# eboigne/PyTV-4D

Measured on AMD Instinct MI355X. Metric: chambolle_pock_iters_per_sec, higher is better.
Workload: dtype f32

## Files before the change

### pytv-4d_amd/csrc/tv_fused.h

```cpp
#pragma once
#include "tv_device.h"
#include "tv_stencil.h"

namespace tv {

using F4 = Vec<float, 4>;

#ifndef TV_FUSED_TR
#define TV_FUSED_TR 8
#endif
#ifndef TV_FUSED_NW
#define TV_FUSED_NW 8
#endif
#ifndef TV_ADMM_T_NT
#define TV_ADMM_T_NT 0
#endif
#ifndef TV_FUSED_PFQ_TWIN
#define TV_FUSED_PFQ_TWIN 1
#endif
#ifndef TV_FUSED_PFQ
#define TV_FUSED_PFQ 2
#endif
#ifndef TV_FUSED_PFX
#define TV_FUSED_PFX 1
// ... 644 lines not shown
    return vload_s<T, V>(p);
#else
    return vload<T, V>(p);
#endif
}
template <typename T, int V> __device__ __forceinline__ void FXST(T* p, const Vec<T, V>& a) {
#if TV_FIXUP_NT
    vstore_s<T, V>(p, a);
#else
    vstore<T, V>(p, a);
#endif
}
template <int S, bool XW, typename T = float, int ALG = ALG_CP>
__device__ __forceinline__ double fixup_site(const DG& g, const WT<T>& w, const FixupArgsT<T>& a, int zchunk, int zl, int t, int y,
                                             int col0) {
    constexpr int V = 16 / (int)sizeof(T);
    using VT = Vec<T, V>;
    constexpr bool UP = (S != DOWNWIND), DN = (S != UPWIND), CEN = (S == CENTRAL);
    if (!fused_needs_fixup<S, XW, V>(g, zl, y, col0, zchunk, t)) return 0.0;
    constexpr int CM = XW ? CPG<V>::BC - 1 : CPG<V>::WC - 1;
    const int c_ru = 0, c_cu = 1, c_rd = (S == HYBRID) ? 2 : 0, c_cd = (S == HYBRID) ? 3 : 1;
    const int c_zu = g.ch_z, c_zd = (S == HYBRID) ? g.ch_z + 1 : g.ch_z;
    const bool z_fwd = CEN && g.z_two;
    const long long inpl = (long long)t * g.s_t + (long long)y * g.rp + col0;
    const T* qb = a.q + (long long)zl * g.s_dz + inpl;
    const VT zero = vsplat<T, V>(T(0));
    VT m = zero;
    if (UP && (y & (CP_TR - 1)) == 0 && y >= (CEN ? 2 : 1)) m = m + FXLD<T, V>(qb + (long long)c_ru * g.s_z - g.rp);
    if (DN && (y & (CP_TR - 1)) == CP_TR - 1 && y <= g.ny - (CEN ? 3 : 2)) m = m - FXLD<T, V>(qb + (long long)c_rd * g.s_z + g.rp);
    if (UP && (col0 & CM) == 0 && col0 >= (CEN ? 2 : 1)) m.v[0] += qb[(long long)c_cu * g.s_z - 1];
    if (DN && (col0 & CM) == CM - (V - 1) && col0 + V <= g.nx - (CEN ? 2 : 1)) m.v[V - 1] -= qb[(long long)c_cd * g.s_z + V];
    if (g.za) {
        const int gz = g.z0 + zl;
        const int zs = (zl / zchunk) * zchunk;
        const int ze = (zs + zchunk < g.nz) ? zs + zchunk : g.nz;
        if (UP && zl == zs && gz >= ((CEN && !z_fwd) ? 2 : 1)) {
            const VT u = (zl >= 1) ? FXLD<T, V>(qb + (long long)c_zu * g.s_z - g.s_dz) : FXLD<T, V>(a.qp + inpl);
            m = m + w.wz * u;
        }
        if (DN && !z_fwd && zl == ze - 1 && gz <= g.nzg - (CEN ? 3 : 2)) {
            const VT d = (zl + 1 < g.nz) ? FXLD<T, V>(qb + (long long)c_zd * g.s_z + g.s_dz) : FXLD<T, V>(a.qn + inpl);
            m = m - w.wz * d;
        }
    }
    if (g.ta && g.m > CP_TWN) {
        const int c_tu = g.ch_t, c_td = (S == HYBRID) ? g.ch_t + 1 : g.ch_t;
        const int k = t % CP_TWN;
        VT mt = zero;
        if (UP && k == 0 && t >= 1) mt = mt + FXLD<T, V>(qb + (long long)c_tu * g.s_z - g.s_t) * vol_factor<T, V>(g, zl, t - 1, y, col0);
        if (DN && k == CP_TWN - 1 && t <= g.m - (CEN ? 3 : 2))
            mt = mt - FXLD<T, V>(qb + (long long)c_td * g.s_z + g.s_t) * vol_factor<T, V>(g, zl, t + 1, y, col0);
        m = m + (w.wt * mt) * mask_factor<T, V>(g, w.sf, y, col0);
    }
    const T s = (S == HYBRID) ? Consts<T>::inv_sqrt2() : (CEN ? T(0.5) : T(1));
    const long long off = (long long)zl * g.s_z + inpl;
    const VT xv = FXLD<T, V>(a.x_out + off);
    VT x0v = zero;
    if constexpr (ALG == ALG_CP) { if (a.x0 != nullptr) x0v = FXLD<T, V>(a.x0 + off); }
    VT xo;
    double acc = 0.0;
#pragma unroll
    for (int i = 0; i < V; ++i) {
        xo.v[i] = xv.v[i] - a.tau * (s * m.v[i]);
        const double e = (double)xo.v[i] - (double)x0v.v[i];
        acc += (ALG == ALG_CP ? 0.5 : 1.0) * e * e;
    }
    FXST<T, V>(a.x_out + off, xo);
    return acc;
}

template <int S> __device__ __forceinline__ bool is_fix_row(const DG& g, int y) {
    constexpr bool UP = (S != DOWNWIND), DN = (S != UPWIND);
    return (UP && (y & (CP_TR - 1)) == 0 && y >= 1) || (DN && (y & (CP_TR - 1)) == CP_TR - 1 && y <= g.ny - 2);
}
template <int S> __device__ __forceinline__ bool is_fix_plane(const DG& g, int zl, int zchunk) {
    constexpr bool UP = (S != DOWNWIND), DN = (S != UPWIND);
    if (!g.za) return false;
    const int gz = g.z0 + zl;
    const int zs = (zl / zchunk) * zchunk;
    const int ze = (zs + zchunk < g.nz) ? zs + zchunk : g.nz;
    return (UP && zl == zs && gz >= 1) || (DN && zl == ze - 1 && gz <= g.nzg - 2);
}

template <int S, int CLS, bool XW, typename T = float, int ALG = ALG_CP>
__global__ __launch_bounds__(256) void k_cp_fixup(DG g, WT<T> w, FixupArgsT<T> a, int zchunk, int zb, int zn, double* partials) {
    constexpr int V = 16 / (int)sizeof(T);
    __shared__ double sm[16];
    const int nxv = (g.nx + V - 1) / V;
    const int tiles_x = (nxv + 63) / 64;
    double acc = 0.0;
    if (CLS == 0) {
        const int bx = (int)blockIdx.x % tiles_x, grp = (int)blockIdx.x / tiles_x;
        const int ty = (int)threadIdx.y;
        int y;
        if (S == HYBRID || S == CENTRAL) y = grp * 2 * CP_TR + ((ty & 1) ? CP_TR - 1 : 0) + ((ty & 2) ? CP_TR : 0);
        else y = grp * 4 * CP_TR + CP_TR * ty + (S == DOWNWIND ? CP_TR - 1 : 0);
        const int col0 = (bx * 64 + (int)threadIdx.x) * V;
        if (col0 < g.nx && y < g.ny && is_fix_row<S>(g, y) && !is_seam_frame<S>(g, (int)blockIdx.y))
            acc = fixup_site<S, XW, T, ALG>(g, w, a, zchunk, zb + (int)blockIdx.z, (int)blockIdx.y, y, col0);
    } else if (CLS == 1) {
        const int k = (int)blockIdx.z, chunk = a.chunk0 + (k >> 1);
        const int zs = chunk * zchunk;
        const int ze = (zs + zchunk < g.nz) ? zs + zchunk : g.nz;
        const int zl = (k & 1) ? ze - 1 : zs;
        const bool dup = (k & 1) && (ze - 1 == zs);
        const int bx = (int)blockIdx.x % tiles_x, by = (int)blockIdx.x / tiles_x;
        const int y = by * 4 + (int)threadIdx.y;
        const int col0 = (bx * 64 + (int)threadIdx.x) * V;
        if (!dup && zs < g.nz && zl >= zb && zl < zb + zn && col0 < g.nx && y < g.ny && is_fix_plane<S>(g, zl, zchunk) &&
            !is_fix_row<S>(g, y) && !is_seam_frame<S>(g, (int)blockIdx.y))
            acc = fixup_site<S, XW, T, ALG>(g, w, a, zchunk, zl, (int)blockIdx.y, y, col0);
    } else if (CLS == 3) {
        const int wdw = (int)blockIdx.y >> 1, t = wdw * CP_TWN + (((int)blockIdx.y & 1) ? CP_TWN - 1 : 0);
        const int bx = (int)blockIdx.x % tiles_x, by = (int)blockIdx.x / tiles_x;
        const int y = by * 4 + (int)threadIdx.y;
        const int col0 = (bx * 64 + (int)threadIdx.x) * V;
        if (t < g.m && col0 < g.nx && y < g.ny && is_seam_frame<S>(g, t))
            acc = fixup_site<S, XW, T, ALG>(g, w, a, zchunk, zb + (int)blockIdx.z, t, y, col0);
    } else {
        constexpr int TW = XW ? CPG<V>::BC : CPG<V>::WC;
        const int ntile = (g.nx + TW - 1) / TW, ncand = 2 * ntile;
        const long long idx = (long long)blockIdx.x * 256 + (int)threadIdx.y * 64 + (int)threadIdx.x;
        const int zl = zb + (int)blockIdx.z;
        if (idx < (long long)g.ny * ncand && !is_fix_plane<S>(g, zl, zchunk) && !is_seam_frame<S>(g, (int)blockIdx.y)) {
            const int y = (int)(idx / ncand), cnd = (int)(idx % ncand);
            const int col0 = (cnd >> 1) * TW + ((cnd & 1) ? TW - V : 0);
            if (col0 < g.nx && !is_fix_row<S>(g, y)) acc = fixup_site<S, XW, T, ALG>(g, w, a, zchunk, zl, (int)blockIdx.y, y, col0);
        }
    }
    acc = block_sum(acc, sm);
    if (threadIdx.x == 0 && threadIdx.y == 0) partials[linear_block_id()] = acc;
}


template <int S, int M>
__global__ __launch_bounds__(256, 2) void k_subgrad_march(DG g, WT<float> w, const float* __restrict__ x, const float* __restrict__ xp,
                                                          const float* __restrict__ xn, const float* __restrict__ norms_ext,
                                                          float* __restrict__ G, int zchunk) {
    static_assert(S != CENTRAL, "radius-2 scheme");
    constexpr bool UP = (S == UPWIND || S == HYBRID), DN = (S == DOWNWIND || S == HYBRID);
    const FusedCoord c = fused_coord(g, zchunk, 0);
    const F4 zero = vsplat<float, 4>(0.f), one = vsplat<float, 4>(1.f);
    const F4 mf = g.ta ? mask_factor<float, 4>(g, w.sf, c.ok ? c.y : 0, c.ok ? c.col0 : 0) : one;
    __shared__ F4 lds_WC[M][256];
    __shared__ F4 lds_WP[M][256];
    const int tid = (int)threadIdx.y * 64 + (int)threadIdx.x;
    auto nplane = [&](int zl) -> const float* {
        const int gz = g.z0 + zl;
        return (gz >= 0 && gz < g.nzg) ? norms_ext + (long long)(zl + 1) * g.s_z : nullptr;
    };
    F4 XC[M], XP[M];
    {
        const float* pc = zplane<float>(g, x, xp, xn, 2, c.zs);
        const float* pp = g.za ? zplane<float>(g, x, xp, xn, 2, c.zs - 1) : nullptr;
        const float* qc = nplane(c.zs);
        const float* qp = g.za ? nplane(c.zs - 1) : nullptr;
#pragma unroll
        for (int t = 0; t < M; ++t) {
            const long long off = (long long)t * g.s_t + c.inpl;
            XC[t] = c.ok ? vload<float, 4>(pc + off) : zero;
            XP[t] = (c.ok && pp) ? vload<float, 4>(pp + off) : zero;
            lds_WC[t][tid] = c.ok ? vload<float, 4>(qc + off) : one;
            lds_WP[t][tid] = (c.ok && qp && UP) ? vload<float, 4>(qp + off) : one;
        }
    }
    auto neighbourhood = [&](XN<float, 4>& n, const F4& cv, const float* plane_c, long long off, const F4& nzv, const F4& pzv,
                             const F4& ntv, const F4& ptv, bool h_nz, bool h_pz, bool h_nt, bool h_pt) {
        n.c = cv;
        n.col0 = c.col0;
        const bool want_up = (c.row == 0) && c.ok && (c.y > 0);
        const bool want_dn = (c.row == 3) && c.ok && (c.y + 1 < g.ny);
        F4 halo = zero;
        if (want_up || want_dn) halo = vload<float, 4>(plane_c + off + (want_up ? -(long long)g.rp : (long long)g.rp));
        n.h_nr = c.ok && (c.y + 1 < g.ny);
        n.h_pr = c.ok && (c.y > 0);
        const F4 sdn = shfl_down16(cv), sup = shfl_up16(cv);
        n.nr = (c.row == 3) ? halo : sdn;
        n.pr = (c.row == 0) ? halo : sup;
        const bool le = (c.lx == 0) && c.ok && (c.col0 > 0), re = (c.lx == 15) && c.ok && (c.col0 + 4 < g.nx);
        float edge = 0.f;
        if (le || re) edge = le ? plane_c[off - 1] : plane_c[off + 4];
        const float shr = __shfl_down(cv.v[0], 1, 64), shl = __shfl_up(cv.v[3], 1, 64);
        n.nc = shift_left<float, 4>(cv, (c.lx == 15) ? edge : shr);
        n.pc = shift_right<float, 4>(cv, (c.lx == 0) ? edge : shl);
        n.nz = nzv; n.pz = pzv; n.nt = ntv; n.pt = ptv;
        n.h_nz = h_nz; n.h_pz = h_pz; n.h_nt = h_nt; n.h_pt = h_pt;
    };
    for (int z = c.zs; z < c.ze; ++z) {
        const int gz = g.z0 + z;
        const float* pc = zplane<float>(g, x, xp, xn, 2, z);
        const float* pn = zplane<float>(g, x, xp, xn, 2, z + 1);
        const float* qc = nplane(z);
        const float* qn = nplane(z + 1);
        const bool has_pz = g.za && (gz > 0), has_nz = g.za && (pn != nullptr);
        const bool more = (z + 1 < c.ze);
        F4 xcold = zero, wcold = one;
#pragma unroll
        for (int t = 0; t < M; ++t) {
            const long long off = (long long)t * g.s_t + c.inpl;
            const F4 XNv = (pn != nullptr && c.ok && (has_nz || more)) ? vload<float, 4>(pn + off) : zero;
            const F4 WNv = (qn != nullptr && c.ok && ((has_nz && DN) || more)) ? vload<float, 4>(qn + off) : one;
            const F4 wc = lds_WC[t][tid], wp = lds_WP[t][tid];
            const bool h_nt = g.ta && (t + 1 < M), h_pt = g.ta && (t > 0);
            XN<float, 4> xs, ns;
            neighbourhood(xs, XC[t], pc, off, XNv, XP[t], XC[(t + 1 < M) ? t + 1 : t], xcold, has_nz, has_pz, h_nt, h_pt);
            neighbourhood(ns, wc, qc, off, WNv, wp, lds_WC[(t + 1 < M) ? t + 1 : t][tid], wcold, has_nz, has_pz, h_nt, h_pt);
            if (c.ok) {
                const F4 r = subgrad_site<S, float, 4>(g, w, xs, ns, mf);
                vstore<float, 4>(G + (long long)z * g.s_z + off, r);
            }
            xcold = XC[t];
            wcold = wc;
            XP[t] = XC[t];
            XC[t] = XNv;
// ... 8 lines not shown
```

### pytv-4d_amd/csrc/tv_fused.hip

```cpp
#include "tv_fused_launch.h"

TV_FUSED_INSTANTIATE(float, ALG_CP)

static int fused_zchunk(const DG& d) {
    int zc = env_int("TV_ZCHUNK", 0);
    if (zc <= 0) {
        const long long nwin = (d.m > CP_TWN) ? (d.m + CP_TWN - 1) / CP_TWN : 1;
        const long long tiles = (long long)(((d.nx + d.vl - 1) / d.vl + CP_NW * CP_TL - 1) / (CP_NW * CP_TL)) * ((d.ny + CP_TR - 1) / CP_TR) * nwin;
        const long long want = (1024 + tiles - 1) / (tiles > 0 ? tiles : 1);
        zc = (int)(d.nz / (want > 0 ? want : 1));
        if (zc > 32) zc = 32;
        if (zc < 8) zc = 8;
        while (zc > 2 && tiles * ((d.nz + zc - 1) / zc) < 256) zc -= 2;
        if (d.nz < d.nzg) {
            const int q4 = (int)(d.nz / 4);
            if (zc > q4) zc = q4 < 4 ? 4 : q4;
        }
    }
    if (zc < 1) zc = 1;
    if (zc > d.nz) zc = (int)d.nz;
    return zc;
}

namespace tvm {
bool subgrad_pass2_ok(const tv_geom* g, const DG& d) { return g->scheme != TV_CENTRAL && d.m >= 1 && d.m <= 8; }
int subgrad_pass2(const tv_geom* g, const DG& d, const void* x, const void* xp, const void* xn, hipStream_t st,
                  const float* norms_ext, float* G) {
    const int zc = march_zchunk(d);
    const LC lc = march_cfg(d, zc);
    return dispatch_scheme_m(WindowedMs{}, g->scheme, d.m, kNoFusedSM, [&]<int S, int M>() -> int {
        if constexpr (S != CENTRAL && M >= 1) {
            hipLaunchKernelGGL((k_subgrad_march<S, M>), lc.grid, lc.block, 0, st, d, make_w<float>(g), (const float*)x,
                               (const float*)xp, (const float*)xn, norms_ext, G, zc);
            HIP_TRY(hipGetLastError());
            return 0;
        } else {
            return fail(TV_E_ARG, "central: radius-2 gather, not a marching kernel");
        }
    });
}
}

struct SweepPlan {
    LC lc;
    int zc, chunk0;
    bool xw, force_win;
};
static int sweep_plan(const tv_geom* g, const DG& d, const Partials& P, const void* x_in, const void* x_prev, const void* x_next,
                      int64_t chunk_begin, int64_t chunk_count, SweepPlan& sp, bool& empty) {
    sp.zc = fused_zchunk(d);
    const int zc = sp.zc;
    {
        const long long nch_all = (d.nz + zc - 1) / zc;
        const long long cb = (chunk_count < 0) ? 0 : chunk_begin, ce = (chunk_count < 0) ? nch_all : chunk_begin + chunk_count;
        const bool first = (cb == 0 && ce > 0), last = (ce == nch_all && ce > cb);
        if (int rc = check_x_halos(g, d, first ? x_prev : x_in, last ? x_next : x_in)) return rc;
    }
    LC& lc = sp.lc;
    lc = march_cfg(d, zc);
    {
        const long long tx = ((d.nx + d.vl - 1) / d.vl + CP_NW * CP_TL - 1) / (CP_NW * CP_TL), ty = (d.ny + CP_TR - 1) / CP_TR;
        lc.grid.x = (unsigned)(tx * ty);
        lc.block = dim3(64, CP_NW, 1);
        lc.nblocks = tx * ty * lc.grid.y;
    }
    const long long nch = lc.grid.y;
    if (chunk_count < 0) { chunk_begin = 0; chunk_count = nch; }
    if (chunk_begin < 0 || chunk_begin + chunk_count > nch) return fail(TV_E_ARG, "chunk range outside the slab");
    empty = (chunk_count == 0);
    if (empty) return 0;
    const int nwin = (d.m > CP_TWN) ? (d.m + CP_TWN - 1) / CP_TWN : 1;
    lc.grid.y = (unsigned)chunk_count;
    lc.grid.z = (unsigned)nwin;
    lc.nblocks = (long long)lc.grid.x * chunk_count * nwin;
    if (lc.nblocks > P.nmax) return fail(TV_E_ARG, "internal: sweep partials exceed the workspace");
    sp.chunk0 = (int)chunk_begin;
    sp.xw = env_int("TV_FUSED_XW", 1) != 0;
    sp.force_win = (d.m == CP_TWN) && env_int("TV_FUSED_FORCE_TWIN", (g->scheme == TV_HYBRID || g->scheme == TV_CENTRAL) ? 1 : 0);
    return 0;
}

static int fixup_plan(const tv_geom* g, const DG& d, const Partials& P, const void* q, const void* q_prev, const void* q_next, int64_t z_begin,
                      int64_t z_count, FixPlan& fp, bool& empty) {
    const int zc = fused_zchunk(d);
    if (z_count < 0) { z_begin = 0; z_count = d.nz; }
    if (z_begin < 0 || z_begin + z_count > d.nz) return fail(TV_E_ARG, "plane range outside the slab");
    empty = (z_count == 0);
    if (empty) return 0;
    if (int rc = check_y_halos(g, d, (z_begin == 0) ? q_prev : q, (z_begin + z_count == d.nz) ? q_next : q)) return rc;
    const int zb = (int)z_begin, zn = (int)z_count;
    const int chunk_lo = zb / zc, chunk_hi = (zb + zn - 1) / zc;
    const long long tiles_x = ((d.nx + d.vl - 1) / d.vl + 63) / 64, tiles_y = (d.ny + 3) / 4;
    const long long ngrp = (g->scheme == TV_HYBRID || g->scheme == TV_CENTRAL) ? (d.ny + 2 * CP_TR - 1) / (2 * CP_TR)
                                                                                : (d.ny + 4 * CP_TR - 1) / (4 * CP_TR);
    const bool xw = env_int("TV_FUSED_XW", 1) != 0;
    const long long bc = (long long)CP_NW * CP_TL * d.vl, wc = (long long)CP_TL * d.vl;
    const long long ncand = xw ? 2ll * ((d.nx + bc - 1) / bc) : 2ll * ((d.nx + wc - 1) / wc);
    fp.g0 = dim3((unsigned)(tiles_x * ngrp), (unsigned)d.m, (unsigned)zn);
    fp.g1 = dim3((unsigned)(tiles_x * tiles_y), (unsigned)d.m, (unsigned)(2 * (chunk_hi - chunk_lo + 1)));
    fp.g2 = dim3((unsigned)(((long long)d.ny * ncand + 255) / 256), (unsigned)d.m, (unsigned)zn);
    const int nwin = (d.m > CP_TWN && d.ta) ? (d.m + CP_TWN - 1) / CP_TWN : 0;
    fp.g3 = dim3((unsigned)(tiles_x * tiles_y), (unsigned)(2 * (nwin > 0 ? nwin : 1)), (unsigned)zn);
    fp.n0 = (long long)fp.g0.x * fp.g0.y * fp.g0.z;
    fp.n1 = d.za ? (long long)fp.g1.x * fp.g1.y * fp.g1.z : 0;
    fp.n2 = (long long)fp.g2.x * fp.g2.y * fp.g2.z;
    fp.n3 = nwin > 0 ? (long long)fp.g3.x * fp.g3.y * fp.g3.z : 0;
    if (fp.n0 + fp.n1 + fp.n2 + fp.n3 > P.nmax) return fail(TV_E_ARG, "internal: fix-up partials exceed the workspace");
    fp.chunk_lo = chunk_lo; fp.zc = zc; fp.zb = zb; fp.zn = zn; fp.xw = xw;
    return 0;
}

template <int ALG, typename MakeArgs>
static int run_sweep(const tv_geom* g, const DG& d, const void* x_in, const void* x_prev, const void* x_next, int64_t chunk_begin,
                     int64_t chunk_count, void* ws, hipStream_t st, double* tvout, double* sums, int nsum, MakeArgs&& make_args) {
    const Partials P(ws, d);
    SweepPlan sp;
    bool empty = false;
    if (int rc = sweep_plan(g, d, P, x_in, x_prev, x_next, chunk_begin, chunk_count, sp, empty)) return rc;
    if (empty) {
        HIP_TRY(hipMemsetAsync(tvout, 0, sizeof(double), st));
        if (nsum > 0) HIP_TRY(hipMemsetAsync(sums, 0, nsum * sizeof(double), st));
        return 0;
    }
    if (int rc = dispatch_dtype(g->dtype, [&]<typename T>() -> int {
            return tvm::fused_sweep<T, ALG>(g, d, sp.lc, st, make_args.template operator()<T>(P), sp.zc, sp.chunk0, sp.xw, sp.force_win);
        }))
        return rc;
    if (int rc = P.reduce(0, sp.lc.nblocks, tvout, st)) return rc;
    for (int k = 0; k < nsum; ++k)
        if (int rc = P.reduce(1 + k, sp.lc.nblocks, sums + k, st)) return rc;
    return 0;
}

template <int ALG, typename MakeArgs>
static int run_fixup(const tv_geom* g, const DG& d, const void* q, const void* q_prev, const void* q_next, int64_t z_begin, int64_t z_count,
                     Partials P, hipStream_t st, double* out, bool has_sum, MakeArgs&& make_args) {
    FixPlan fp;
    bool empty = false;
    if (int rc = fixup_plan(g, d, P, q, q_prev, q_next, z_begin, z_count, fp, empty)) return rc;
    if (!empty) {
        if (int rc = dispatch_dtype(g->dtype, [&]<typename T>() -> int {
                return tvm::fused_fixup<T, ALG>(g, d, st, make_args.template operator()<T>(fp), fp, P.slot(0));
            }))
            return rc;
        if (has_sum) return P.reduce(0, fp.n0 + fp.n1 + fp.n2 + fp.n3, out, st);
    }
    HIP_TRY(hipMemsetAsync(out, 0, sizeof(double), st));
    return 0;
}

extern "C" {

int tv_cp_fused_supported(const tv_geom* g) {
    DG d;
    if (make_dg(g, d, true)) return 0;
    if ((!d.pitched && d.nx % d.vl != 0) || d.nx < 64) return 0;
    if (d.m > CP_TWN && env_int("TV_NO_FUSED_TWIN", 0)) return 0;
    if (d.s_t * (16 / d.vl) >= (1ll << 31)) return 0;
    if (env_int("TV_NO_FUSED", 0)) return 0;
    return 1;
}

int tv_cp_zchunk(const tv_geom* g) {
    DG d;
    if (int rc = make_dg(g, d, true)) return rc;
    return fused_zchunk(d);
}

static int cp_sweep_impl(const tv_geom* g, const void* x_in, const void* x_prev, const void* x_next, const void* q_in, void* q, const void* x0,
                         void* p, void* x_out, double sigma_D, double lambda, double tau, double sigma_A, int32_t flags, int64_t chunk_begin,
                         int64_t chunk_count, double* tvout, double* fid, void* ws, void* stream) {
    DG d;
    if (int rc = make_dg(g, d, true)) return rc;
    if (!x_in || !q || !x0 || !p || !x_out || !tvout || !fid || !ws) return fail(TV_E_ARG, "NULL array");
    if (x_in == x_out) return fail(TV_E_ARG, "x_in and x_out must be different buffers (ping-pong)");
    if (!(lambda > 0.0)) return fail(TV_E_ARG, "lambda must be > 0");
    if (!tv_cp_fused_supported(g)) return fail(TV_E_ARG, "geometry not supported by the one-sweep path");
    if (!aligned16({x_in, x_prev, x_next, q, x0, p, x_out, d.wv})) return fail(TV_E_ARG, "arrays must be 16-byte aligned");
    auto args = [&]<typename T>(const Partials& P) {
        return FusedArgsT<T>{(const T*)x_in, (const T*)x_prev, (const T*)x_next, (T*)q, (const T*)x0, (T*)p,
                             (T*)x_out, (T)sigma_D, (T)(1.0 / lambda), (T)tau, (T)sigma_A, (T)(1.0 / (1.0 + sigma_A)), P.slot(0), P.slot(1),
                             ((flags & TV_CP_FID_OF_INPUT) ? 2 : 0) | ((flags & TV_CP_FID_BOTH) ? 4 : 0), (const T*)(q_in ? q_in : q), P.slot(2)};
    };
    return run_sweep<ALG_CP>(g, d, x_in, x_prev, x_next, chunk_begin, chunk_count, ws, (hipStream_t)stream, tvout, fid,
                             (flags & TV_CP_FID_BOTH) ? 2 : 1, args);
}

int tv_cp_fused(const tv_geom* g, const void* x_in, const void* x_prev, const void* x_next, void* q, const void* x0,
                void* p, void* x_out, double sigma_D, double lambda, double tau, double sigma_A, int64_t chunk_begin,
                int64_t chunk_count, double* tvout, double* fid, void* ws, void* stream) {
// ... 93 lines not shown
```

### pytv-4d_amd/csrc/tv_fused_launch.h

```cpp
#pragma once
#include "tv_host.h"
#include "tv_stencil.h"
#include "tv_fused.h"

struct FixPlan {
    dim3 g0, g1, g2, g3;
    long long n0, n1, n2, n3;
    int chunk_lo, zc, zb, zn;
    bool xw;
};

inline constexpr const char* kNoFusedSM = "unsupported (scheme, M) for the one-sweep path";

template <typename T, int ALG>
static int fused_sweep_launch(const tv_geom* g, const DG& d, const LC& lc, hipStream_t st, const FusedArgsT<T>& a, int zc, int chunk0, bool xw,
                              bool force_win) {
    if (ALG != ALG_CP && !xw) return fail(TV_E_ARG, "the ADMM / operator sweeps are built with TV_FUSED_XW=1 only");
    return dispatch_scheme_m(WindowedMs{}, g->scheme, (d.m > CP_TWN || force_win) ? 0 : d.m, kNoFusedSM, [&]<int S, int M>() -> int {
        if constexpr (M == 0) {
            if (xw) hipLaunchKernelGGL((k_cp_fused<S, CP_TWN, true, true, T, ALG>), lc.grid, lc.block, 0, st, d, make_w<T>(g), a, zc, chunk0);
            else if constexpr (ALG == ALG_CP)
                hipLaunchKernelGGL((k_cp_fused<S, CP_TWN, false, true, T, ALG>), lc.grid, lc.block, 0, st, d, make_w<T>(g), a, zc, chunk0);
        } else if (xw) hipLaunchKernelGGL((k_cp_fused<S, M, true, false, T, ALG>), lc.grid, lc.block, 0, st, d, make_w<T>(g), a, zc, chunk0);
        else if constexpr (ALG == ALG_CP)
            hipLaunchKernelGGL((k_cp_fused<S, M, false, false, T, ALG>), lc.grid, lc.block, 0, st, d, make_w<T>(g), a, zc, chunk0);
        HIP_TRY(hipGetLastError());
        return 0;
    });
}

template <typename T, int ALG>
static int fused_fixup_launch(const tv_geom* g, const DG& d, hipStream_t st, const FixupArgsT<T>& a, const FixPlan& p, double* w0) {
    if (ALG != ALG_CP && !p.xw) return fail(TV_E_ARG, "the ADMM / operator sweeps are built with TV_FUSED_XW=1 only");
    const dim3 blk(64, 4, 1);
    return dispatch_scheme(g->scheme, [&]<int S>() -> int {
        auto launch = [&]<bool XW>() -> int {
            if constexpr (ALG == ALG_CP || XW) {
                hipLaunchKernelGGL((k_cp_fixup<S, 0, XW, T, ALG>), p.g0, blk, 0, st, d, make_w<T>(g), a, p.zc, p.zb, p.zn, w0);
                if (d.za) hipLaunchKernelGGL((k_cp_fixup<S, 1, XW, T, ALG>), p.g1, blk, 0, st, d, make_w<T>(g), a, p.zc, p.zb, p.zn, w0 + p.n0);
                hipLaunchKernelGGL((k_cp_fixup<S, 2, XW, T, ALG>), p.g2, blk, 0, st, d, make_w<T>(g), a, p.zc, p.zb, p.zn, w0 + p.n0 + p.n1);
                if (p.n3 > 0)
                    hipLaunchKernelGGL((k_cp_fixup<S, 3, XW, T, ALG>), p.g3, blk, 0, st, d, make_w<T>(g), a, p.zc, p.zb, p.zn, w0 + p.n0 + p.n1 + p.n2);
                HIP_TRY(hipGetLastError());
            }
            return 0;
        };
        return p.xw ? launch.template operator()<true>() : launch.template operator()<false>();
    });
}

namespace tvm {
template <typename T, int ALG>
int fused_sweep(const tv_geom* g, const DG& d, const LC& lc, hipStream_t st, const FusedArgsT<T>& a, int zc, int chunk0, bool xw, bool force_win);
template <typename T, int ALG> int fused_fixup(const tv_geom* g, const DG& d, hipStream_t st, const FixupArgsT<T>& a, const FixPlan& p, double* w0);
}

#define TV_FUSED_INSTANTIATE(T, ALG)                                                                                                       \
    namespace tvm {                                                                                                                        \
    template <>                                                                                                                            \
    int fused_sweep<T, ALG>(const tv_geom* g, const DG& d, const LC& lc, hipStream_t st, const FusedArgsT<T>& a, int zc, int chunk0, bool xw, \
                            bool force_win) {                                                                                              \
        return fused_sweep_launch<T, ALG>(g, d, lc, st, a, zc, chunk0, xw, force_win);                                                     \
    }                                                                                                                                      \
    template <> int fused_fixup<T, ALG>(const tv_geom* g, const DG& d, hipStream_t st, const FixupArgsT<T>& a, const FixPlan& p, double* w0) { \
        return fused_fixup_launch<T, ALG>(g, d, st, a, p, w0);                                                                             \
    }                                                                                                                                      \
    }
```

### pytv-4d_amd/csrc/tv_host.h

```cpp
#pragma once
#include <hip/hip_runtime.h>

#include <atomic>
#include <cassert>
#include <cmath>
#include <cstdio>
#include <cstdlib>
#include <cstring>
#include <initializer_list>
#include <mutex>
#include <string>
#include <utility>

#include "../../include/pytv4d.h"
#include "tv_device.h"

using namespace tv;

namespace tv { __global__ void k_reduce(const double* in, long long n, double* out); }

inline thread_local std::string g_err;
inline int fail(int code, const char* msg) {
    g_err = msg;
    return code;
// ... 87 lines not shown
inline long long max_partials(const DG& d) {
    LC lc = launch_cfg(d, 1, d.nz + 2);
    const long long tiles = (long long)(((d.nx + 3) / (d.vl > 0 ? d.vl : 4) + 63) / 64 + 1) * ((d.ny + 3) / 4 + 1);
    long long n = 4 * tiles * (d.m + 2) * (d.nz + 2) + 4096;
    if (lc.nblocks > n) n = lc.nblocks;
    return n > kFlatBlocks ? n : kFlatBlocks;
}

struct Partials {
    double* base;
    long long nmax;
    static constexpr int kSlots = 3;
    Partials(void* ws, const DG& d) : base((double*)ws), nmax(max_partials(d)) {}
    long long slot_words() const { return nmax + kStage + 16; }
    static size_t bytes(const DG& d) { return (size_t)(kSlots * Partials(nullptr, d).slot_words()) * sizeof(double); }
    double* slot(int k) const { return base + k * slot_words(); }
    double* spare(int k, int i = 0) const {
        assert(k >= 1 && k < kSlots && i >= -16 && i <= 1);
        return slot(k) + i;
    }
    int reduce(int k, long long n, double* result, hipStream_t st) const {
        if (n > nmax) return fail(TV_E_ARG, "internal: partials exceed the workspace");
        double* const w = slot(k);
        if (n <= 4096) {
            hipLaunchKernelGGL(k_reduce, dim3(1), dim3(256), 0, st, w, n, result);
        } else {
            double* stage = w + nmax;
            hipLaunchKernelGGL(k_reduce, dim3(kStage), dim3(256), 0, st, w, n, stage);
            hipLaunchKernelGGL(k_reduce, dim3(1), dim3(256), 0, st, stage, (long long)kStage, result);
        }
        HIP_TRY(hipGetLastError());
        return 0;
    }
};

inline bool aligned16(std::initializer_list<const void*> ps) {
    for (const void* p : ps)
        if (p != nullptr && (reinterpret_cast<uintptr_t>(p) & 15u) != 0) return false;
    return true;
}

inline int vec_lanes(const tv_geom* g) { return g->dtype == TV_F32 ? 4 : 2; }
inline bool rows_vectorisable(const tv_geom* g, const DG& d) { return d.pitched || d.nx % vec_lanes(g) == 0; }

template <typename F> inline int dispatch_scheme(int scheme, F&& f) {
    switch (scheme) {
        case UPWIND: return f.template operator()<UPWIND>();
        case DOWNWIND: return f.template operator()<DOWNWIND>();
        case CENTRAL: return f.template operator()<CENTRAL>();
        case HYBRID: return f.template operator()<HYBRID>();
    }
    return fail(TV_E_ARG, "unknown scheme");
}
template <typename F> inline int dispatch_dtype(int dtype, F&& f) {
    return (dtype == TV_F32) ? f.template operator()<float>() : f.template operator()<double>();
}
template <typename F> inline int dispatch(int scheme, int dtype, bool vec, F&& f) {
    return dispatch_scheme(scheme, [&]<int S>() -> int {
        return dispatch_dtype(dtype, [&]<typename T>() -> int {
            constexpr int L = 16 / (int)sizeof(T);
            return vec ? f.template operator()<S, T, L>() : f.template operator()<S, T, 1>();
        });
    });
}
using MarchMs = std::integer_sequence<int, 1, 2, 3, 4, 5, 6, 7, 8, 16>;
using WindowedMs = std::integer_sequence<int, 0, 1, 2, 3, 4, 5, 6, 7, 8>;
template <int... Ms, typename F> inline int dispatch_m(std::integer_sequence<int, Ms...>, int m, const char* what, F&& f) {
    int rc = 0;
    const bool hit = ((m == Ms && ((rc = f.template operator()<Ms>()), true)) || ...);
    return hit ? rc : fail(TV_E_ARG, what);
}
template <typename Ms, typename F> inline int dispatch_scheme_m(Ms ms, int scheme, int m, const char* what, F&& f) {
    return dispatch_scheme(scheme, [&]<int S>() -> int {
        return dispatch_m(ms, m, what, [&]<int M>() -> int { return f.template operator()<S, M>(); });
    });
}

struct TvOption { const char* name; std::atomic<int> has; std::atomic<int> value; };
inline TvOption g_options[] = {
    {"TV_NO_MARCH", 0, 0}, {"TV_MARCH_MIN_PLANE_KB", 0, 0}, {"TV_ZCHUNK", 0, 0}, {"TV_NS_ZCHUNK", 0, 0}, {"TV_MARCH_D", 0, 0},
    {"TV_NO_MARCH_SUBGRAD", 0, 0}, {"TV_NO_MARCH_NORMAL", 0, 0}, {"TV_SCALAR_GATHER", 0, 0}, {"TV_NO_FUSED", 0, 0},
    {"TV_NO_FUSED_TWIN", 0, 0}, {"TV_FUSED_XW", 0, 0}, {"TV_FUSED_FORCE_TWIN", 0, 0}, {"TV_NO_FUSED_SUBGRAD", 0, 0},
    {"TV_NORMAL_KERNEL", 0, 0}, {"TV_D_KERNEL", 0, 0}, {"TV_DT_KERNEL", 0, 0}, {"TV_FUSED_MIN_KVOXELS", 0, 0}, {"TV_SG_KERNEL", 0, 0}, {"TV_SPARE", 0, 0}, {"TV_SG_ALIGNED", 0, 0},
    {"TV_SMALL_MAX_KVOXELS", 0, 0}, {"TV_NO_SMALL", 0, 0}, {"TV_SMALL_BLOCKS_PER_CU", 0, 0}, {"TV_SMALL_GENERIC", 0, 0}, {"TV_SMALL_TILES", 0, 0}, {"TV_SMALL_SITES", 0, 0}, {"TV_NS_NO_FIRST", 0, 0},
};
inline std::once_flag g_options_once;
inline TvOption* find_option(const char* name) {
    std::call_once(g_options_once, [] {
        for (TvOption& o : g_options) {
            const char* v = getenv(o.name);
            if (v && *v) { o.value = atoi(v); o.has = 1; }
        }
    });
    for (TvOption& o : g_options)
        if (strcmp(o.name, name) == 0) return &o;
    return nullptr;
}
inline int env_int(const char* name, int dflt) {
    const TvOption* o = find_option(name);
    return (o && o->has.load(std::memory_order_relaxed)) ? o->value.load(std::memory_order_relaxed) : dflt;
}
inline bool plane_big_enough(const DG& d, int elt) {
    return (long long)d.s_z * elt >= (long long)env_int("TV_MARCH_MIN_PLANE_KB", 4096) * 1024;
}
inline bool march_geom_ok(const DG& d, bool vec, int elt) {
    if (!vec || d.nx < 128) return false;
    if (d.wv != nullptr) return false;
    if (d.pitched) return false;
    if (env_int("TV_NO_MARCH", 0)) return false;
    if (!plane_big_enough(d, elt)) return false;
    return (d.m >= 1 && d.m <= 8) || d.m == 16;
}
inline bool march_ok(const tv_geom* g, const DG& d, bool vec) { return g->dtype == TV_F32 && march_geom_ok(d, vec, 4); }
inline bool march_dt_ok(const tv_geom* g, const DG& d, bool vec, bool plain_store) {
    if (g->dtype == TV_F32) return march_ok(g, d, vec) && !(plain_store && (g->scheme == TV_UPWIND || g->scheme == TV_DOWNWIND));
    return g->scheme == TV_HYBRID && plain_store && march_geom_ok(d, vec, 8);
}
inline int march_zchunk(const DG& d) {
    int zc = env_int("TV_ZCHUNK", 0);
    if (zc <= 0) {
        long long tiles = (long long)((d.nx / d.vl + 63) / 64) * ((d.ny + 3) / 4);
        if (tiles < 1) tiles = 1;
        const long long want_chunks = (4096 + tiles - 1) / tiles;
        zc = (int)(d.nz / (want_chunks > 0 ? want_chunks : 1));
        if (zc > 32) zc = 32;
        if (zc < 4) zc = 4;
    }
    if (zc < 1) zc = 1;
    if (zc > d.nz) zc = d.nz;
    return zc;
}
inline LC march_cfg(const DG& d, int zchunk) {
    const long long tx = (d.nx / d.vl + 63) / 64, ty = (d.ny + 3) / 4, nch = (d.nz + zchunk - 1) / zchunk;
    LC lc;
    lc.block = dim3(64, 4, 1);
    lc.grid = dim3((unsigned)(tx * ty), (unsigned)nch, 1);
    lc.nblocks = tx * ty * nch;
    return lc;
}
inline constexpr const char* kNoMarchSM = "unsupported (scheme, M) for the marching path";
inline int check_x_halos(const tv_geom* g, const DG& d, const void* xp, const void* xn) {
    if (!d.za) return 0;
    const bool need_prev = (g->scheme != TV_UPWIND), need_next = (g->scheme != TV_DOWNWIND);
    if (need_prev && g->z0 > 0 && xp == nullptr) return fail(TV_E_HALO, "previous-slab halo plane required");
    if (need_next && g->z0 + g->nz < g->nz_global && xn == nullptr) return fail(TV_E_HALO, "next-slab halo plane required");
    return 0;
}
inline int check_x_halos2(const tv_geom* g, const DG& d, const void* x_prev, const void* x_next, const char* who) {
    const bool e_lo = (g->z0 > 0), e_hi = (g->z0 + g->nz < g->nz_global);
    if (d.za && ((e_lo && x_prev == nullptr) || (e_hi && x_next == nullptr))) {
        g_err = std::string(who) + " on a slab needs two halo planes on each interior side";
        return TV_E_HALO;
    }
    return 0;
}
inline int check_y_halos(const tv_geom* g, const DG& d, const void* yp, const void* yn) {
    if (!d.za) return 0;
    const bool need_prev = (g->scheme != TV_DOWNWIND), need_next = (g->scheme != TV_UPWIND);
    if (need_prev && g->z0 > 0 && yp == nullptr) return fail(TV_E_HALO, "previous-slab gradient halo required");
    if (need_next && g->z0 + g->nz < g->nz_global && yn == nullptr) return fail(TV_E_HALO, "next-slab gradient halo required");
    return 0;
}

namespace tvm {
int D_store(const tv_geom* g, const DG& d, const void* x, const void* xp, const void* xn, hipStream_t st, long long* nb, float* dout);
int D_cp_dual(const tv_geom* g, const DG& d, const void* x, const void* xp, const void* xn, hipStream_t st, long long* nb,
              float* q, float sigma, float inv_lambda, double* partials);
// ... 26 lines not shown
```

Measured before the change: 30.09.

## Merge four fix-up class launches into one interleaved grid launch

Replaces the up-to-four separate k_cp_fixup launches (row, plane, column and seam-frame classes) with a single launch. The block index is decoded into a class and a per-class block id through a FixGrid table, with classes interleaved in groups so they are spread across the grid. This removes per-launch overhead and the tail idle time between small dependent-free kernels. In exchange, every block pays for runtime class decoding, the kernel is no longer specialised per class at compile time (more divergent code and possibly higher register use), and some blocks exit early as padding.

```diff
diff --git a/pytv-4d_amd/csrc/tv_fused.h b/pytv-4d_amd/csrc/tv_fused.h
--- a/pytv-4d_amd/csrc/tv_fused.h
+++ b/pytv-4d_amd/csrc/tv_fused.h
@@ -750,54 +750,78 @@
     return (UP && zl == zs && gz >= 1) || (DN && zl == ze - 1 && gz <= g.nzg - 2);
 }
 
-template <int S, int CLS, bool XW, typename T = float, int ALG = ALG_CP>
-__global__ __launch_bounds__(256) void k_cp_fixup(DG g, WT<T> w, FixupArgsT<T> a, int zchunk, int zb, int zn, double* partials) {
+struct FixGrid {
+    unsigned gx[4], gy[4];
+    unsigned n[4];
+    unsigned per[4];
+    unsigned pg;
+};
+
+template <int S, bool XW, typename T = float, int ALG = ALG_CP>
+__global__ __launch_bounds__(256) void k_cp_fixup(DG g, WT<T> w, FixupArgsT<T> a, int zchunk, int zb, int zn, FixGrid fg, double* partials) {
     constexpr int V = 16 / (int)sizeof(T);
     __shared__ double sm[16];
+    const unsigned grp = blockIdx.x / fg.pg, r = blockIdx.x % fg.pg;
+    const unsigned e0 = fg.per[0], e1 = e0 + fg.per[1], e2 = e1 + fg.per[2];
+    const int cls = (int)(r >= e0) + (int)(r >= e1) + (int)(r >= e2);
+    const unsigned start = (cls == 0) ? 0u : (cls == 1) ? e0 : (cls == 2) ? e1 : e2;
+    const unsigned per = (cls == 0) ? fg.per[0] : (cls == 1) ? fg.per[1] : (cls == 2) ? fg.per[2] : fg.per[3];
+    const unsigned ncl = (cls == 0) ? fg.n[0] : (cls == 1) ? fg.n[1] : (cls == 2) ? fg.n[2] : fg.n[3];
+    const unsigned gx = (cls == 0) ? fg.gx[0] : (cls == 1) ? fg.gx[1] : (cls == 2) ? fg.gx[2] : fg.gx[3];
+    const unsigned gy = (cls == 0) ? fg.gy[0] : (cls == 1) ? fg.gy[1] : (cls == 2) ? fg.gy[2] : fg.gy[3];
+    const unsigned long long id = (unsigned long long)grp * per + (r - start);
+    if (id >= ncl) return;
+    const long long pbase = (cls == 0) ? 0ll : (cls == 1) ? (long long)fg.n[0] : (cls == 2) ? (long long)fg.n[0] + fg.n[1]
+                                                                                              : (long long)fg.n[0] + fg.n[1] + fg.n[2];
+    const int bx_ = (int)((unsigned)id % gx), by_ = (int)(((unsigned)id / gx) % gy), bz_ = (int)(((unsigned)id / gx) / gy);
+
     const int nxv = (g.nx + V - 1) / V;
     const int tiles_x = (nxv + 63) / 64;
-    double acc = 0.0;
-    if (CLS == 0) {
-        const int bx = (int)blockIdx.x % tiles_x, grp = (int)blockIdx.x / tiles_x;
+    bool on = false;
+    int zl = 0, t = by_, y = 0, col0 = 0;
+    if (cls == 0) {
+        const int bx = bx_ % tiles_x, rg = bx_ / tiles_x;
         const int ty = (int)threadIdx.y;
-        int y;
-        if (S == HYBRID || S == CENTRAL) y = grp * 2 * CP_TR + ((ty & 1) ? CP_TR - 1 : 0) + ((ty & 2) ? CP_TR : 0);
-        else y = grp * 4 * CP_TR + CP_TR * ty + (S == DOWNWIND ? CP_TR - 1 : 0);
-        const int col0 = (bx * 64 + (int)threadIdx.x) * V;
-        if (col0 < g.nx && y < g.ny && is_fix_row<S>(g, y) && !is_seam_frame<S>(g, (int)blockIdx.y))
-            acc = fixup_site<S, XW, T, ALG>(g, w, a, zchunk, zb + (int)blockIdx.z, (int)blockIdx.y, y, col0);
-    } else if (CLS == 1) {
-        const int k = (int)blockIdx.z, chunk = a.chunk0 + (k >> 1);
+        if (S == HYBRID || S == CENTRAL) y = rg * 2 * CP_TR + ((ty & 1) ? CP_TR - 1 : 0) + ((ty & 2) ? CP_TR : 0);
+        else y = rg * 4 * CP_TR + CP_TR * ty + (S == DOWNWIND ? CP_TR - 1 : 0);
+        col0 = (bx * 64 + (int)threadIdx.x) * V;
+        zl = zb + bz_;
+        on = col0 < g.nx && y < g.ny && is_fix_row<S>(g, y) && !is_seam_frame<S>(g, t);
+    } else if (cls == 1) {
+        const int chunk = a.chunk0 + (bz_ >> 1);
         const int zs = chunk * zchunk;
         const int ze = (zs + zchunk < g.nz) ? zs + zchunk : g.nz;
-        const int zl = (k & 1) ? ze - 1 : zs;
-        const bool dup = (k & 1) && (ze - 1 == zs);
-        const int bx = (int)blockIdx.x % tiles_x, by = (int)blockIdx.x / tiles_x;
-        const int y = by * 4 + (int)threadIdx.y;
-        const int col0 = (bx * 64 + (int)threadIdx.x) * V;
-        if (!dup && zs < g.nz && zl >= zb && zl < zb + zn && col0 < g.nx && y < g.ny && is_fix_plane<S>(g, zl, zchunk) &&
-            !is_fix_row<S>(g, y) && !is_seam_frame<S>(g, (int)blockIdx.y))
-            acc = fixup_site<S, XW, T, ALG>(g, w, a, zchunk, zl, (int)blockIdx.y, y, col0);
-    } else if (CLS == 3) {
-        const int wdw = (int)blockIdx.y >> 1, t = wdw * CP_TWN + (((int)blockIdx.y & 1) ? CP_TWN - 1 : 0);
-        const int bx = (int)blockIdx.x % tiles_x, by = (int)blockIdx.x / tiles_x;
-        const int y = by * 4 + (int)threadIdx.y;
-        const int col0 = (bx * 64 + (int)threadIdx.x) * V;
-        if (t < g.m && col0 < g.nx && y < g.ny && is_seam_frame<S>(g, t))
-            acc = fixup_site<S, XW, T, ALG>(g, w, a, zchunk, zb + (int)blockIdx.z, t, y, col0);
+        zl = (bz_ & 1) ? ze - 1 : zs;
+        const bool dup = (bz_ & 1) && (ze - 1 == zs);
+        const int bx = bx_ % tiles_x, by = bx_ / tiles_x;
+        y = by * 4 + (int)threadIdx.y;
+        col0 = (bx * 64 + (int)threadIdx.x) * V;
+        on = !dup && zs < g.nz && zl >= zb && zl < zb + zn && col0 < g.nx && y < g.ny && is_fix_plane<S>(g, zl, zchunk) &&
+             !is_fix_row<S>(g, y) && !is_seam_frame<S>(g, t);
+    } else if (cls == 3) {
+        const int wdw = by_ >> 1;
+        t = wdw * CP_TWN + ((by_ & 1) ? CP_TWN - 1 : 0);
+        const int bx = bx_ % tiles_x, by = bx_ / tiles_x;
+        y = by * 4 + (int)threadIdx.y;
+        col0 = (bx * 64 + (int)threadIdx.x) * V;
+        zl = zb + bz_;
+        on = t < g.m && col0 < g.nx && y < g.ny && is_seam_frame<S>(g, t);
     } else {
         constexpr int TW = XW ? CPG<V>::BC : CPG<V>::WC;
         const int ntile = (g.nx + TW - 1) / TW, ncand = 2 * ntile;
-        const long long idx = (long long)blockIdx.x * 256 + (int)threadIdx.y * 64 + (int)threadIdx.x;
-        const int zl = zb + (int)blockIdx.z;
-        if (idx < (long long)g.ny * ncand && !is_fix_plane<S>(g, zl, zchunk) && !is_seam_frame<S>(g, (int)blockIdx.y)) {
-            const int y = (int)(idx / ncand), cnd = (int)(idx % ncand);
-            const int col0 = (cnd >> 1) * TW + ((cnd & 1) ? TW - V : 0);
-            if (col0 < g.nx && !is_fix_row<S>(g, y)) acc = fixup_site<S, XW, T, ALG>(g, w, a, zchunk, zl, (int)blockIdx.y, y, col0);
-        }
-    }
+        const long long idx = (long long)bx_ * 256 + (int)threadIdx.y * 64 + (int)threadIdx.x;
+        zl = zb + bz_;
+        if (idx < (long long)g.ny * ncand && !is_fix_plane<S>(g, zl, zchunk) && !is_seam_frame<S>(g, t)) {
+            y = (int)(idx / ncand);
+            const int cnd = (int)(idx % ncand);
+            col0 = (cnd >> 1) * TW + ((cnd & 1) ? TW - V : 0);
+            on = col0 < g.nx && !is_fix_row<S>(g, y);
+        }
+    }
+    double acc = 0.0;
+    if (on) acc = fixup_site<S, XW, T, ALG>(g, w, a, zchunk, zl, t, y, col0);
     acc = block_sum(acc, sm);
-    if (threadIdx.x == 0 && threadIdx.y == 0) partials[linear_block_id()] = acc;
+    if (threadIdx.x == 0 && threadIdx.y == 0) partials[pbase + (long long)id] = acc;
 }
 
 
diff --git a/pytv-4d_amd/csrc/tv_fused.hip b/pytv-4d_amd/csrc/tv_fused.hip
--- a/pytv-4d_amd/csrc/tv_fused.hip
+++ b/pytv-4d_amd/csrc/tv_fused.hip
@@ -96,16 +96,34 @@
     const bool xw = env_int("TV_FUSED_XW", 1) != 0;
     const long long bc = (long long)CP_NW * CP_TL * d.vl, wc = (long long)CP_TL * d.vl;
     const long long ncand = xw ? 2ll * ((d.nx + bc - 1) / bc) : 2ll * ((d.nx + wc - 1) / wc);
-    fp.g0 = dim3((unsigned)(tiles_x * ngrp), (unsigned)d.m, (unsigned)zn);
-    fp.g1 = dim3((unsigned)(tiles_x * tiles_y), (unsigned)d.m, (unsigned)(2 * (chunk_hi - chunk_lo + 1)));
-    fp.g2 = dim3((unsigned)(((long long)d.ny * ncand + 255) / 256), (unsigned)d.m, (unsigned)zn);
     const int nwin = (d.m > CP_TWN && d.ta) ? (d.m + CP_TWN - 1) / CP_TWN : 0;
-    fp.g3 = dim3((unsigned)(tiles_x * tiles_y), (unsigned)(2 * (nwin > 0 ? nwin : 1)), (unsigned)zn);
-    fp.n0 = (long long)fp.g0.x * fp.g0.y * fp.g0.z;
-    fp.n1 = d.za ? (long long)fp.g1.x * fp.g1.y * fp.g1.z : 0;
-    fp.n2 = (long long)fp.g2.x * fp.g2.y * fp.g2.z;
-    fp.n3 = nwin > 0 ? (long long)fp.g3.x * fp.g3.y * fp.g3.z : 0;
-    if (fp.n0 + fp.n1 + fp.n2 + fp.n3 > P.nmax) return fail(TV_E_ARG, "internal: fix-up partials exceed the workspace");
+    const long long cg[4][3] = {{tiles_x * ngrp, d.m, zn},
+                                {tiles_x * tiles_y, d.m, d.za ? 2 * (chunk_hi - chunk_lo + 1) : 0},
+                                {((long long)d.ny * ncand + 255) / 256, d.m, zn},
+                                {tiles_x * tiles_y, 2 * nwin, zn}};
+    long long n[4], total = 0;
+    for (int c = 0; c < 4; ++c) total += (n[c] = cg[c][0] * cg[c][1] * cg[c][2]);
+    fp.n0 = n[0]; fp.n1 = n[1]; fp.n2 = n[2]; fp.n3 = n[3];
+    if (total > P.nmax) return fail(TV_E_ARG, "internal: fix-up partials exceed the workspace");
+    long long groups = env_int("TV_FIXUP_GROUPS", 0);
+    if (groups <= 0) {
+        groups = total;
+        for (int c = 0; c < 4; ++c)
+            if (n[c] > 0 && n[c] < groups) groups = n[c];
+    }
+    if (groups > total) groups = total;
+    long long pg = 0;
+    for (int c = 0; c < 4; ++c) {
+        const long long per = (n[c] + groups - 1) / groups;
+        fp.fg.gx[c] = (unsigned)(cg[c][0] > 0 ? cg[c][0] : 1);
+        fp.fg.gy[c] = (unsigned)(cg[c][1] > 0 ? cg[c][1] : 1);
+        fp.fg.n[c] = (unsigned)n[c];
+        fp.fg.per[c] = (unsigned)per;
+        pg += per;
+    }
+    if (groups * pg >= (1ll << 31)) return fail(TV_E_ARG, "internal: fix-up grid too large");
+    fp.fg.pg = (unsigned)pg;
+    fp.grid = dim3((unsigned)(groups * pg), 1, 1);
     fp.chunk_lo = chunk_lo; fp.zc = zc; fp.zb = zb; fp.zn = zn; fp.xw = xw;
     return 0;
 }
diff --git a/pytv-4d_amd/csrc/tv_fused_launch.h b/pytv-4d_amd/csrc/tv_fused_launch.h
--- a/pytv-4d_amd/csrc/tv_fused_launch.h
+++ b/pytv-4d_amd/csrc/tv_fused_launch.h
@@ -4,7 +4,8 @@
 #include "tv_fused.h"
 
 struct FixPlan {
-    dim3 g0, g1, g2, g3;
+    dim3 grid;
+    FixGrid fg;
     long long n0, n1, n2, n3;
     int chunk_lo, zc, zb, zn;
     bool xw;
@@ -36,11 +37,7 @@
     return dispatch_scheme(g->scheme, [&]<int S>() -> int {
         auto launch = [&]<bool XW>() -> int {
             if constexpr (ALG == ALG_CP || XW) {
-                hipLaunchKernelGGL((k_cp_fixup<S, 0, XW, T, ALG>), p.g0, blk, 0, st, d, make_w<T>(g), a, p.zc, p.zb, p.zn, w0);
-                if (d.za) hipLaunchKernelGGL((k_cp_fixup<S, 1, XW, T, ALG>), p.g1, blk, 0, st, d, make_w<T>(g), a, p.zc, p.zb, p.zn, w0 + p.n0);
-                hipLaunchKernelGGL((k_cp_fixup<S, 2, XW, T, ALG>), p.g2, blk, 0, st, d, make_w<T>(g), a, p.zc, p.zb, p.zn, w0 + p.n0 + p.n1);
-                if (p.n3 > 0)
-                    hipLaunchKernelGGL((k_cp_fixup<S, 3, XW, T, ALG>), p.g3, blk, 0, st, d, make_w<T>(g), a, p.zc, p.zb, p.zn, w0 + p.n0 + p.n1 + p.n2);
+                hipLaunchKernelGGL((k_cp_fixup<S, XW, T, ALG>), p.grid, blk, 0, st, d, make_w<T>(g), a, p.zc, p.zb, p.zn, p.fg, w0);
                 HIP_TRY(hipGetLastError());
             }
             return 0;
diff --git a/pytv-4d_amd/csrc/tv_host.h b/pytv-4d_amd/csrc/tv_host.h
--- a/pytv-4d_amd/csrc/tv_host.h
+++ b/pytv-4d_amd/csrc/tv_host.h
@@ -193,7 +193,7 @@
     {"TV_NO_MARCH_SUBGRAD", 0, 0}, {"TV_NO_MARCH_NORMAL", 0, 0}, {"TV_SCALAR_GATHER", 0, 0}, {"TV_NO_FUSED", 0, 0},
     {"TV_NO_FUSED_TWIN", 0, 0}, {"TV_FUSED_XW", 0, 0}, {"TV_FUSED_FORCE_TWIN", 0, 0}, {"TV_NO_FUSED_SUBGRAD", 0, 0},
     {"TV_NORMAL_KERNEL", 0, 0}, {"TV_D_KERNEL", 0, 0}, {"TV_DT_KERNEL", 0, 0}, {"TV_FUSED_MIN_KVOXELS", 0, 0}, {"TV_SG_KERNEL", 0, 0}, {"TV_SPARE", 0, 0}, {"TV_SG_ALIGNED", 0, 0},
-    {"TV_SMALL_MAX_KVOXELS", 0, 0}, {"TV_NO_SMALL", 0, 0}, {"TV_SMALL_BLOCKS_PER_CU", 0, 0}, {"TV_SMALL_GENERIC", 0, 0}, {"TV_SMALL_TILES", 0, 0}, {"TV_SMALL_SITES", 0, 0}, {"TV_NS_NO_FIRST", 0, 0},
+    {"TV_SMALL_MAX_KVOXELS", 0, 0}, {"TV_NO_SMALL", 0, 0}, {"TV_SMALL_BLOCKS_PER_CU", 0, 0}, {"TV_SMALL_GENERIC", 0, 0}, {"TV_SMALL_TILES", 0, 0}, {"TV_SMALL_SITES", 0, 0}, {"TV_NS_NO_FIRST", 0, 0}, {"TV_FIXUP_GROUPS", 0, 0},
 };
 inline std::once_flag g_options_once;
 inline TvOption* find_option(const char* name) {
```

Result: no change. 30.09 (-0.0%).
